# r-mafi/ClaraGenomicsAnalysis

Measured on AMD Instinct MI355X. Metric: POA windows/sec (consensus), higher is better.
Workload: dtype int16

## Files before the change

claragenomicsanalysis_amd/csrc/poa_batch.cpp:

```cpp
#include <claraparabricks/genomeworks/cudapoa/batch.hpp>
#include <claraparabricks/genomeworks/cudapoa/utils.hpp>

#include "gwamd_cudapoa.h"
#include "host_common.hpp"
#include "poa_batch_internal.hpp"
#include "poa_common.hpp"
#include "poa_plan.hpp"

#include <hip/hip_runtime.h>

#include <algorithm>
#include <cstdio>
#include <cstdlib>
#include <cstring>
#include <iomanip>
#include <sstream>
#include <string>

extern "C" hipError_t gwamd_internal_poa_launch(const gwamd::poa::Buffers* b, const gwamd::poa::Dims* d,
                                       const gwamd::poa::Scores* sc, int score_bits, int size_bits, int banded,
                                       int msa, hipStream_t stream);
extern "C" int gwamd_internal_poa_blocks_per_cu(const gwamd::poa::Dims* d, int score_bits, int size_bits, int banded,
                                                int msa);
extern "C" gwamd::poa::KernelRef gwamd_internal_poa_kernel(const gwamd::poa::Dims* d, int score_bits, int size_bits,
// ... 112 lines not shown
    }

    StatusType add_poa_group(std::vector<StatusType>& per_seq_status, const Group& poa_group) override
    {
        int32_t max_len = 0;
        for (const auto& e : poa_group)
            max_len = std::max(max_len, e.length);
        if (!reserve_buf(max_len))
            return StatusType::exceeded_maximum_poas;
        per_seq_status.clear();
        StatusType st = add_poa();
        if (st != StatusType::success)
            return st;
        for (const auto& e : poa_group)
            per_seq_status.push_back(add_seq_to_poa(e.seq, e.weights, e.length));
        return StatusType::success;
    }

    int32_t get_total_poas() const override { return poa_count_; }

    void generate_poa() override
    {
        if (poa_count_ == 0)
            return;
        upload();
        launch();
    }

    void upload()
    {
        ScopedDevice dev(device_id_);
        const size_t nb = num_bases_;
        GWAMD_HIP_CHECK(hipMemcpyAsync(d_seqs_.data(), h_seqs_.as<uint8_t>(), nb + 16, hipMemcpyHostToDevice, stream_));
        GWAMD_HIP_CHECK(hipMemcpyAsync(d_wts_.data(), h_wts_.as<int8_t>(), nb + 16, hipMemcpyHostToDevice, stream_));
        GWAMD_HIP_CHECK(hipMemcpyAsync(d_len_.data(), h_len_.as<int32_t>(), size_t(num_seqs_) * 4,
                                       hipMemcpyHostToDevice, stream_));
        GWAMD_HIP_CHECK(hipMemcpyAsync(d_off_.data(), h_off_.as<int64_t>(), size_t(num_seqs_) * 8,
                                       hipMemcpyHostToDevice, stream_));
        GWAMD_HIP_CHECK(hipMemcpyAsync(d_win_.data(), h_win_.as<gwamd::poa::WindowDesc>(),
                                       size_t(poa_count_) * sizeof(gwamd::poa::WindowDesc), hipMemcpyHostToDevice,
                                       stream_));
        bufs_.order = nullptr;
        bufs_.head  = nullptr;
        const auto kind = gwamd::poa::plan_window_order(h_win_.as<gwamd::poa::WindowDesc>(), h_len_.as<int32_t>(),
                                                        poa_count_, order_cus_, cap_.slots, dims_.lds_kernel != 0,
                                                        order_);
        if (kind == gwamd::poa::kNoOrder)
            return;
        const size_t order_b = size_t(poa_count_) * 4;
        h_order_.reserve(order_b, stream_);
        std::memcpy(h_order_.as<int32_t>(), order_.data(), order_b);
        int32_t* d_order = reinterpret_cast<int32_t*>(d_win_.data() + lay_.order_off);
        GWAMD_HIP_CHECK(hipMemcpyAsync(d_order, h_order_.as<int32_t>(), order_b, hipMemcpyHostToDevice, stream_));
        bufs_.order = d_order;
        if (kind == gwamd::poa::kOrderAndHead)
            bufs_.head = reinterpret_cast<int32_t*>(d_win_.data() + lay_.head_off);
    }

    void launch()
    {
        if (poa_count_ == 0)
            return;
        ScopedDevice dev(device_id_);
        gwamd::poa::Buffers b = bufs_;
        b.num_windows         = poa_count_;
        b.num_slots           = cap_.slots;
        if (b.head)
// ... 156 lines not shown

    void get_graphs(std::vector<DirectedGraph>& graphs, std::vector<StatusType>& output_status) override
    {
        fetch_graphs();
        graphs.resize(poa_count_);
        const size_t mn = size_t(dims_.max_nodes);
        for (int32_t w = 0; w < poa_count_; w++)
        {
            StatusType st = graph_status(w);
            output_status.push_back(st);
            if (st != StatusType::success)
                continue;
            DirectedGraph& g = graphs[w];
            for (int32_t v = 0; v < h_final_nodes_[w]; v++)
            {
                g.set_node_label(v, std::string(1, char(h_g_bases_[w * mn + v])));
                const int ne = h_g_in_cnt_[w * mn + v];
                for (int e = 0; e < ne; e++)
                {
                    size_t idx = (w * mn + v) * gwamd::poa::kMaxEdges + e;
                    g.add_edge(h_g_in_e_[idx], v, h_g_in_w_[idx]);
                }
            }
        }
    }

    int32_t batch_id() const override { return bid_; }

    void reset() override
    {
        poa_count_          = 0;
        num_bases_          = 0;
        num_seqs_           = 0;
        next_scores_offset_ = 0;
        avail_scorebuf_     = cap_.scorebuf_alloc;
        generated_          = false;
    }

    int32_t score_bits() const { return score_bits_; }
    int32_t size_bits() const { return size_bits_; }
    const gwamd::poa::Dims& dims() const { return dims_; }
    const std::vector<uint8_t>& host_cons() const { return h_cons_; }
    const std::vector<uint16_t>& host_cov() const { return h_cov_; }
    const std::vector<int32_t>& host_cons_len() const { return h_len_out_; }
    const std::vector<uint8_t>& host_status() const { return h_status_; }
    const std::vector<uint8_t>& host_msa() const { return h_msa_; }
    const std::vector<int32_t>& host_msa_len() const { return h_msa_len_; }
    const std::vector<uint8_t>& host_msa_status() const { return h_msa_status_; }
    const std::vector<uint8_t>& host_g_bases() const { return h_g_bases_; }
    const std::vector<uint16_t>& host_g_in_cnt() const { return h_g_in_cnt_; }
    const std::vector<int32_t>& host_g_in_e() const { return h_g_in_e_; }
    const std::vector<uint16_t>& host_g_in_w() const { return h_g_in_w_; }
    const std::vector<int32_t>& host_final_nodes() const { return h_final_nodes_; }
    int32_t window_num_seqs(int32_t w) const { return h_win_.as<const gwamd::poa::WindowDesc>()[w].num_seqs; }
    int8_t output_mask() const { return output_mask_; }
    int64_t device_bytes() const { return lay_.device_bytes(); }
    int32_t kernel_kind() const
    {
        return dims_.lds_kernel == 3 ? (dims_.band_ad ? 4 : 3) : (dims_.lds_kernel ? 2 : 1);
    }
    int32_t max_poas() const { return cap_.max_poas; }
    int32_t max_sequence_size() const { return bs_.max_sequence_size; }
    int32_t slots() const { return cap_.slots; }
    int32_t resident_slots() const { return cap_.resident; }
    void set_spoa_accurate(bool on) { dims_.spoa_accurate = on ? 1 : 0; }
    bool spoa_accurate() const { return dims_.spoa_accurate != 0; }
// ... 80 lines not shown
        return true;
    }

    StatusType add_poa()
    {
        if (poa_count_ == cap_.max_poas)
            return StatusType::exceeded_maximum_poas;
        h_win_.reserve(size_t(poa_count_ + 1) * sizeof(gwamd::poa::WindowDesc), stream_);
        gwamd::poa::WindowDesc& wd = h_win_.as<gwamd::poa::WindowDesc>()[poa_count_];
        wd.first_seq               = num_seqs_;
        wd.num_seqs                = 0;
        h_win_.used_               = size_t(poa_count_ + 1) * sizeof(gwamd::poa::WindowDesc);
        poa_count_++;
        generated_ = false;
        return StatusType::success;
    }

    StatusType add_seq_to_poa(const char* seq, const int8_t* weights, int32_t seq_len)
    {
        if (seq_len > bs_.max_sequence_size)
            return StatusType::exceeded_maximum_sequence_size;
        gwamd::poa::WindowDesc& wd = h_win_.as<gwamd::poa::WindowDesc>()[poa_count_ - 1];
        if (wd.num_seqs >= bs_.max_sequences_per_poa)
            return StatusType::exceeded_maximum_sequences_per_poa;
        if (weights != nullptr)
            for (int32_t i = 0; i < seq_len; i++)
                detail::check_non_negative(weights[i], "Base weights need to be non-negative");
        wd.num_seqs++;
        const size_t need = num_bases_ + size_t(seq_len) + 16;
        h_seqs_.reserve(need, stream_);
        h_wts_.reserve(need, stream_);
        if (seq_len > 0)
            std::memcpy(h_seqs_.as<uint8_t>() + num_bases_, seq, size_t(seq_len));
        if (weights == nullptr)
            std::memset(h_wts_.as<int8_t>() + num_bases_, 1, size_t(seq_len));
        else if (seq_len > 0)
            std::memcpy(h_wts_.as<int8_t>() + num_bases_, weights, size_t(seq_len));
        std::memset(h_seqs_.as<uint8_t>() + num_bases_ + seq_len, 0, 16);
        std::memset(h_wts_.as<int8_t>() + num_bases_ + seq_len, 0, 16);
        h_len_.reserve(size_t(num_seqs_ + 1) * 4, stream_);
        h_off_.reserve(size_t(num_seqs_ + 1) * 8, stream_);
        h_len_.as<int32_t>()[num_seqs_] = seq_len;
        h_off_.as<int64_t>()[num_seqs_] = int64_t(num_bases_);
        num_bases_ += size_t(seq_len);
        h_seqs_.used_ = h_wts_.used_ = num_bases_ + 16;
        num_seqs_++;
        h_len_.used_ = size_t(num_seqs_) * 4;
        h_off_.used_ = size_t(num_seqs_) * 8;
        return StatusType::success;
    }

    int32_t device_id_;
    hipStream_t stream_;
    int8_t output_mask_;
    BatchSize bs_;
    int16_t gap_, mismatch_, match_;
    bool banded_;
    int32_t score_bits_ = 16, size_bits_ = 16;
    gwamd::poa::PoaCapacity cap_;
    gwamd::poa::PoaLayout lay_;
    int32_t order_cus_ = 0;
    int64_t avail_scorebuf_ = 0, next_scores_offset_ = 0;
    int32_t poa_count_  = 0;
    int32_t num_seqs_   = 0;
    size_t num_bases_   = 0;
    bool generated_     = false;
    int32_t bid_        = 0;
    hipEvent_t ev_start_ = nullptr, ev_stop_ = nullptr;
    const gwamd::poa::PoaTuning tune_ = gwamd::poa::read_poa_tuning();
    gwamd::poa::Dims dims_{};
    std::vector<int32_t> order_;
    PinnedBuf h_order_;
    gwamd::poa::Buffers bufs_{};
    gwamd::host::DevBuf<uint8_t> d_seqs_, d_wts_, d_len_, d_off_, d_win_, d_slab_, d_codes_;
    PinnedBuf h_seqs_, h_wts_, h_len_, h_off_, h_win_;
    std::vector<uint8_t> h_cons_, h_status_, h_msa_, h_msa_status_, h_g_bases_, h_g_in_e_raw_;
    std::vector<uint16_t> h_cov_, h_g_in_cnt_, h_g_in_w_;
    std::vector<int32_t> h_len_out_, h_msa_len_, h_g_in_e_, h_final_nodes_;
    static int32_t batches_;
};

int32_t PoaBatch::batches_ = 0;

StatusType Init()
{
    int n = 0;
    if (hipGetDeviceCount(&n) != hipSuccess || n == 0)
        return StatusType::generic_error;
    return StatusType::success;
}

int64_t estimate_max_poas(const BatchSize& batch_size, bool banded_alignment, bool msa_flag,
                          size_t free_device_memory, float memory_usage_quota, int32_t mismatch_score,
                          int32_t gap_score, int32_t match_score)
{
    const size_t mem_per_batch = size_t(memory_usage_quota * double(free_device_memory));
    int64_t sizeof_score       = 2;
    int64_t per_poa            = 0;
// ... 625 lines not shown
```

claragenomicsanalysis_amd/csrc/poa_common.hpp:

```cpp
#pragma once

#include <cstddef>
#include <cstdint>

#include "poa_handover.hpp"

namespace gwamd
{
namespace poa
{

constexpr int kMaxEdges      = 50;
constexpr int kMaxAlignments = 50;
constexpr int kBandPad       = 8;
constexpr int kWave          = 64;
constexpr int kCellsPerLane  = 8;
constexpr int kChunk         = kWave * kCellsPerLane;
constexpr int kAdRing        = 128;
constexpr int kAdSpillDist   = kAdRing - kWave + 1;
constexpr int band_ring_rows(int cpl) { return cpl >= 16 ? 8 : 16; }
constexpr int band_tile_rows(int cpl) { return cpl >= 10 ? 32 : 64; }
constexpr int kReadGuard     = 64;
constexpr int kAdMaxWaves    = 4;
constexpr int kColShift      = 7;
// ... 34 lines not shown
    int32_t lds_bytes;
    int32_t lds_ring_off;
    int32_t lds_ring_rows;
    int32_t lds_sh_off;
    int32_t lds_rec_off;
    int32_t lds_xl_off;
    int32_t lds_xl_cap;
    int32_t lds_cpl;
    int32_t lds_waves;
    int32_t code_stride;
    int64_t aux_stride;
    int32_t aux_carry_off;
    int32_t lds_work_bytes;
    int32_t aux_reca_off;
    int32_t aux_recb_off;
    int32_t aux_col0_off;
    int32_t aux_flag_off;
    int32_t aux_xl_off;
    int32_t aux_xl_cap;
    int32_t aux_bx_off;
    int32_t aux_recc_off;
    int32_t aux_rece_off;
    int32_t band_ad;
    int32_t tb_rank;
    int32_t diag;
};

constexpr int kTbRanked     = 1;
constexpr int kTbStrips     = 2;
constexpr int kTbStrip32    = 4;
constexpr int kTbDefault    = kTbRanked | kTbStrips;
constexpr int kTbAboveShift = 3;
constexpr int kTbAboveMask  = 7;

constexpr int kDiagTopsortRing  = 1;
constexpr int kDiagFwdV1        = 2;
constexpr int kDiagTopsortFifo  = 4;
constexpr int kDiagRaconV1      = 8;
constexpr int kDiagConsensusHbm = 16;
constexpr int kDiagAddWave0     = 32;
constexpr int kDiagAddSerial    = 64;
constexpr int kDiagOrderKahn    = 128;
constexpr int kDiagSinkCap2     = 256;
constexpr int kDiagConsLdsShift = 16;

struct LdsShape
{
    int cpl, waves;
    bool wide;
};
constexpr LdsShape kLdsShapes[] = {{8, 1, true},   {8, 2, true},   {8, 4, true},   {8, 8, true},  {16, 8, true},
                                   {8, 1, false},  {16, 1, false}, {24, 1, false}, {32, 1, false}, {8, 2, false},
                                   {8, 3, false},  {8, 4, false},  {16, 4, false}, {4, 4, false}};
constexpr int kNumLdsShapes = int(sizeof(kLdsShapes) / sizeof(kLdsShapes[0]));

struct KernelRef
{
    const void* fn;
    int threads;
    size_t dynamic_lds;
};

constexpr int64_t lds_read_bytes(int64_t max_seq_len) { return (max_seq_len + 48 + 15) & ~int64_t(15); }

constexpr int kAddShBytes = 64;
constexpr int64_t lds_add_ms(int64_t max_seq_len) { return (max_seq_len + 16) & ~int64_t(15); }
// ... 121 lines not shown
```

claragenomicsanalysis_amd/csrc/poa_kernels.hip:

```cpp
#include <hip/hip_runtime.h>

#include <climits>
#include <cstdint>
#include <type_traits>
#include <utility>

#include "poa_wave.hpp"
#include "poa_order.hpp"
#include "poa_rowprog.hpp"

namespace gwamd
{
namespace poa
{

template <typename ScoreT, typename SizeT, bool BANDED, bool MSA>
__global__ void __launch_bounds__(kWave) poa_window_kernel(Buffers b, Dims d, Scores sc)
{
    extern __shared__ __align__(16) uint8_t lds_read[];
    __shared__ int sh_alen;
    __shared__ int sh_status;
    __shared__ int sh_len;

    const int w = b.order ? b.order[blockIdx.x] : int(blockIdx.x);
    if (w >= b.num_windows)
        return;
    const int lane = threadIdx.x;

    const WinGraph<SizeT> g     = bind_window<SizeT>(b, d.max_nodes, size_t(w));
    const SlotScratch<SizeT> sl = bind_slot<SizeT>(b, d, size_t(w));
    const WinMsa<SizeT> msa     = bind_window_msa<SizeT, MSA>(b, d, size_t(w));
    ScoreT* S       = static_cast<ScoreT*>(b.scores) + size_t(w) * d.score_rows * size_t(d.score_stride);
    SizeT *ag = sl.ag, *ar = sl.ar, *cpred = sl.cpred, *seq_begin = msa.seq_begin;
    int32_t* cscore = sl.cscore;
    uint16_t *ecov = msa.ecov, *ecovc = msa.ecov_cnt;

    PhaseTimer ph;
    const WindowDesc wd = b.windows[w];
    const int nseq      = wd.num_seqs;
    int status          = kSuccess;
    int64_t cells       = 0;
    int node_count      = 0;
// ... 658 lines not shown
                    if (2 * i + 1 == own_c)
                        endv = int(int16_t(E[i] >> 16));
                }
                const int v = L == 0 ? cin : __builtin_amdgcn_readlane(endv, own_lane);
                if (best_val < v)
                    best_val = v, best_row = r;
            }
#pragma unroll
            for (int i = 0; i < NR; i++)
                Eprev[i] = E[i];
            cin_prev = cin;
            rec_c    = rec_a;
            np_c     = np_a;
            pv_c     = pv_a;
            rec_a    = rec_b;
            np_a     = np_b;
            pv_a     = pv_b;
            rec_b    = uniform(int(rec_bb));
            GWAMD_FP_LAP(fp, 3);
        }
    }
    }
    if (nsweep > 1 || NW > 1)
    {
        GWAMD_LDS int* endp = (GWAMD_LDS int*)(shb + kShEnd);
        if (wave == own_span % NW && lane == 0)
            *endp = best_row;
        __syncthreads();
        best_row = uniform(*endp);
    }
    return best_row;
}

template <typename SizeT>
__device__ int traceback_codes(WinGraph<SizeT> g, const RowProg& P, int V, int L, int end_row,
                               const uint8_t* codes_f, int code_stride, uint8_t* tile_f, SizeT* ag_f, SizeT* ar_f,
                               int aln_cap, int lane, bool rank, int tbmode)
{
    g = as_global(g);
    const GWAMD_GLB uint8_t* codes = glb_of(codes_f);
    GWAMD_LDS uint8_t* tile        = lds_of(tile_f);
    GWAMD_GLB SizeT* ag            = glb_of(ag_f);
    GWAMD_GLB SizeT* ar            = glb_of(ar_f);
    const GWAMD_LDS uint32_t* prec = lds_of(P.rec);
    const GWAMD_LDS uint16_t* pxl  = lds_of(P.xl);

    V       = uniform(V);
    L       = uniform(L);
    int i   = uniform(end_row), j = L;
    int ti0 = INT_MIN / 2, tj0 = INT_MIN / 2;
    int n = 0, loops = 0;
    const int bound = L + V + 2;
    int eg = 0, er = 0;
    auto flush = [&](int upto) { tb_flush<SizeT>(g.sorted, ag, ar, aln_cap, upto, lane, eg, er); };
    auto load_tile = [&](int ii, int cj) {
        ti0 = max(0, ii - (kTileRows - 1));
        tj0 = max(0, cj - (kTileCols - 16)) & ~15;
        wave_sync();
        constexpr int kPer = kTileRows * (kTileCols / 16) / kWave;
        constexpr int kB   = 8;
#pragma unroll
        for (int b0 = 0; b0 < kPer; b0 += kB)
        {
            u32x4 v[kB];
#pragma unroll
            for (int u = 0; u < kB; u++)
            {
                const int t   = (b0 + u) * kWave + lane;
                const int tr  = t / (kTileCols / 16);
                const int tc  = (t % (kTileCols / 16)) * 16;
                const int rr  = ti0 + tr;
                const bool ok = rr <= V && tj0 + tc + 16 <= code_stride;
                v[u] = *reinterpret_cast<const GWAMD_GLB u32x4*>(codes + size_t(ok ? rr : 0) * code_stride +
                                                                 (ok ? tj0 + tc : 0));
                v[u] = ok ? v[u] : u32x4{0, 0, 0, 0};
            }
#pragma unroll
            for (int u = 0; u < kB; u++)
            {
                const int t  = (b0 + u) * kWave + lane;
                const int tr = t / (kTileCols / 16);
                const int tc = (t % (kTileCols / 16)) * 16;
                *reinterpret_cast<GWAMD_LDS u32x4*>(tile + tr * kTileCols + tc) = v[u];
            }
        }
        wave_sync();
    };
    constexpr uint32_t kSlow = 0xffffffffu;
    const bool win_ok        = V < 65535 && L < 65535;
    TbWin G;
    G.init(tbmode, i, L, kTileRows);
    uint32_t wpk0 = kSlow, wpk1 = kSlow;
    auto decode_cell = [&](int t) -> uint32_t {
        const int r  = G.row(t);
        const int c  = G.col(t);
        const int cj = c + kColShift;
        uint32_t res = kSlow;
        if (r >= 1 && c >= 0 && r >= ti0 && r < ti0 + kTileRows && cj >= tj0 && cj < tj0 + kTileCols)
        {
            const int code     = int(tile[(r - ti0) * kTileCols + (cj - tj0)]);
            const uint32_t rec = prec[r];
            const int dir      = code & 3;
            const int np       = int((rec >> 8) & 63);
            const int pj       = dir == 1 ? c : c - 1;
            if (pj < 0)
                res = kSlow;
            else if (dir == 2)
                res = (uint32_t(r) << 16) | uint32_t(pj);
            else if (np != int(kRecEscape))
            {
                const int p = np == 0 ? 0 : (np == 1 ? r - int(rec >> 16) : int(pxl[(rec >> 16) + (code >> 2)]));
                res         = (uint32_t(p) << 16) | uint32_t(pj);
            }
        }
        return res;
    };
    while (!(i == 0 && j == 0) && loops < bound)
    {
        i     = uniform(i);
// ... 50 lines not shown
            const int rec_v    = int(prec[i]);
            const int code     = uniform(code_v);
            const uint32_t rec = uint32_t(uniform(rec_v));
            const int dir      = code & 3;
            if (dir == 2)
            {
                pi = i;
                pj = j - 1;
            }
            else
            {
                const int np = int((rec >> 8) & 63), k = code >> 2;
                pi = np == 0 ? 0
                             : (np == 1 ? i - int(rec >> 16)
                                        : (np == int(kRecEscape) ? uniform(pred_row(g, int(g.sorted[i - 1]), k))
                                                                 : uniform(int(pxl[(rec >> 16) + k]))));
                pj = dir == 0 ? j - 1 : j;
            }
        }
        if (lane == (n & (kWave - 1)))
        {
            eg = i == pi ? -1 : i;
            er = j == pj ? -1 : j - 1;
        }
        n++;
        if ((n & (kWave - 1)) == 0)
            flush(n);
        i = pi;
        j = pj;
    }
    if ((n & (kWave - 1)) != 0)
        flush(n);
    wave_sync();
    if (loops >= bound || n > aln_cap)
        return -1;
    return n;
}

#include "poa_fwd2.hpp"
#include "poa_fwd_w.hpp"

template <bool MSA, int CPL, int NW, bool W>
__global__ void __launch_bounds__(kWave * NW, W ? (NW >= 8 ? 2 : 1) : (NW >= 4 ? 2 : 1))
    poa_window_kernel_lds(Buffers b, Dims d, Scores sc)
{
    using SizeT  = int16_t;
    using RowT   = typename std::conditional<W, int32_t, int16_t>::type;
    extern __shared__ __align__(16) uint8_t lds[];
    __shared__ int sh_status;
    __shared__ int sh_len;

    __shared__ int sh_next;
    if (int(blockIdx.x) >= b.num_windows)
        return;
    const int tid      = threadIdx.x;
    const int lane     = tid & (kWave - 1);
    const int wave     = uniform(tid / kWave);
    constexpr int kThr = kWave * NW;
    const size_t slot  = blockIdx.x;

    uint8_t* lread   = lds;
    RowT* ring       = reinterpret_cast<RowT*>(lds + d.lds_ring_off);
    uint8_t* tile    = lds + d.lds_ring_off;
    const int rstride = d.score_stride;
    GWAMD_LDS uint8_t* shb = (GWAMD_LDS uint8_t*)(lds) + d.lds_sh_off;
    const AddScratch AX = lds_add_scratch((GWAMD_LDS uint8_t*)(lds) + d.lds_ring_off, d.max_seq_len, d.max_nodes,
                                          false, (GWAMD_LDS int*)(shb));
    const bool add_fits = lds_add_fits(d.max_seq_len, d.max_nodes, d.lds_rec_off - d.lds_ring_off);
    const int add_mode  = (d.diag & kDiagAddSerial) ? 2 : (((d.diag & kDiagAddWave0) || !add_fits) ? 1 : 0);

    for (int idx = blockIdx.x; idx < b.num_windows;)
    {
    const int w     = b.order ? b.order[idx] : idx;
    const WinGraph<SizeT> g     = bind_window<SizeT>(b, d.max_nodes, size_t(w));
    const SlotScratch<SizeT> sl = bind_slot<SizeT>(b, d, slot);
    const WinMsa<SizeT> msa     = bind_window_msa<SizeT, MSA>(b, d, size_t(w));
    SizeT *ag = sl.ag, *ar = sl.ar, *cpred = sl.cpred, *seq_begin = msa.seq_begin;
    int32_t* cscore = sl.cscore;
    uint16_t *ecov = msa.ecov, *ecovc = msa.ecov_cnt;
    RowT* spill      = static_cast<RowT*>(b.scores) + slot * d.score_rows * size_t(rstride);
    uint8_t* codes   = b.codes + slot * size_t(d.aux_stride);
    uint32_t* rec    = reinterpret_cast<uint32_t*>(lds + d.lds_rec_off);
    uint16_t* xl     = reinterpret_cast<uint16_t*>(lds + d.lds_xl_off);
    RowT* carry      = reinterpret_cast<RowT*>(codes + d.aux_carry_off);
    RowProg P{rec, xl, d.lds_ring_rows - 1};

    PhaseTimer ph;
    FwdProf fp;
    const bool use_v2 = !W && fwd2_ok(sc) && !(d.diag & kDiagFwdV1);
    const WindowDesc wd = b.windows[w];
    const int nseq      = wd.num_seqs;
    int status          = kSuccess;
    int64_t cells       = 0;
    int node_count      = 0;
    int lv_hint         = 0;
    bool order_kahn = true;
    bool splice_on  = !d.spoa_accurate && !(d.diag & (kDiagTopsortFifo | kDiagOrderKahn));
    int tie_hold    = 0;
    const int sink_cap = (d.diag & kDiagSinkCap2) ? 2 : kSinkCap;
    const int xcap  = d.lds_xl_cap - kSinkWords;
    GWAMD_LDS uint16_t* sinks = (GWAMD_LDS uint16_t*)(lds + d.lds_xl_off) + xcap;
    int32_t* ostat  = b.order_stats + size_t(w) * kOrderStats;
    auto count      = [&](int k) {
        if (tid == 0)
            __hip_atomic_fetch_add(ostat + k, 1, __ATOMIC_RELAXED, __HIP_MEMORY_SCOPE_AGENT);
    };
    if (tid < kOrderStats)
        ostat[tid] = 0;
    auto kahn_sort = [&](WinGraph<SizeT> gx, int n, int n_prev) {
        const bool done = topsort_levels<SizeT, NW>(gx, n, n_prev, (GWAMD_LDS uint8_t*)(lds), d.lds_sh_off, tid,
                                                    kThr, cpred, lv_hint);
        if (!done && tid == 0)
            topsort_kahn<SizeT>(gx, n, cscore);
        lv_hint = done ? n : 0;
        __syncthreads();
    };

    if (nseq > 0)
    {
        const int len0      = b.seq_len[wd.first_seq];
        const uint8_t* seq0 = b.seqs + b.seq_off[wd.first_seq];
// ... 125 lines not shown
                if (code == 2 && !order_kahn)
                {
                    const size_t mn    = size_t(d.max_nodes);
                    WinGraph<SizeT> gk = g;
                    gk.sorted          = cpred + mn;
                    gk.pos             = cpred + 2 * mn;
                    for (int i = tid; i < V; i += kThr)
                        glb(gk.sorted)[i] = glb(g.sorted)[i];
                    kahn_sort(gk, V, V);
                    count(kOsTieSorts);
                    if (wave == 0)
                    {
                        int kp = INT_MAX;
                        if (tied)
                            kp = int(glb(gk.pos)[int(glb(g.sorted)[srow_l - 1])]);
                        const int kmin = -wave_max(-kp);
                        const uint64_t m = __builtin_amdgcn_ballot_w64(kp == kmin);
                        const int er   = __builtin_amdgcn_readlane(srow_l, uniform(__builtin_ctzll(m)));
                        if (lane == 0)
                            sh_len = er;
                    }
                    __syncthreads();
                    end_row = uniform(sh_len);
                    __syncthreads();
                    stage_and_program_w0();
                    __syncthreads();
                }
                tie_hold = code == 2 ? 2 : max(tie_hold - 1, 0);
            }
            else if (tie_hold > 0)
                tie_hold--;
            if (wave == 0)
            {
                const int alen_w = traceback_codes<SizeT>(g, P, V, L, end_row, codes, d.code_stride, tile, ag, ar,
                                                          d.aln_cap, lane, (d.tb_rank & kTbRanked) != 0,
                                                          d.tb_rank);
                if (lane == 0)
                    sh_len = alen_w;
            }
            __syncthreads();
            const int alen = uniform(sh_len);
            __syncthreads();
            ph.lap<kPhTraceback>();
            if (alen == -1)
            {
                status = kLoopCountExceeded;
                break;
            }
            int add_r = -1;
            if (add_mode == 0)
                add_r = add_alignment_waves<MSA, NW, NW + (W ? 16 : 0)>(lds_kernel_args(), w, int(slot), s, off,
                                                                        node_count, alen, L,
                                                                        (GWAMD_LDS uint8_t*)(lds));
            if (wave == 0)
            {
                int nc = node_count;
                int rc = -1;
                if (add_mode == 0)
                {
                    nc = add_r >> 8;
                    rc = (add_r & 0xff) == 0xff ? -1 : (add_r & 0xff);
                }
                else if (add_mode == 1)
                    rc = add_alignment_parallel<SizeT, MSA>(g, nc, ag, ar, alen, L, lread, wts_g, s, ecov, ecovc,
                                                            seq_begin, d.max_seqs, AX, lane);
                if (rc < 0)
                {
                    if (lane == 0)
                    {
// ... 65 lines not shown
                }
                ph.lap<kPhTopsort>();
                wave_sync();
                if (lane == 0)
                {
                    sh_status = rc;
                    sh_len    = nc;
                }
            }
            __syncthreads();
            status     = uniform(sh_status);
            node_count = uniform(sh_len);
            __syncthreads();
            if (status != kSuccess)
                break;
        }
    }
    if (wave == 0)
    {
        finish_window<SizeT, MSA, NW>(b, d, w, lane, g, status, nseq, node_count, cscore, cpred, ecov, ecovc,
                                      seq_begin, sh_len, sh_status, (GWAMD_LDS uint8_t*)(lds), d.lds_sh_off);
        ph.lap<kPhOutput>();
        if (lane == 0)
        {
            if (b.phase)
            {
                ph.store(b.phase + size_t(w) * kPhases);
#ifdef GWAMD_FWD_PROFILE
                const int slot[8] = {kPhBackbone, kPhAdd, kPhTopsort, kPhOutput, kPhForward, kPhTraceback, kPhRowProg,
                                     kPhTotal};
                for (int i = 0; i < 8; i++)
                    b.phase[size_t(w) * kPhases + slot[i]] = int64_t(fp.t[i]);
#endif
            }
            b.final_nodes[w] = node_count;
            b.cells[w]       = cells;
        }
    }
#if defined(GWAMD_FWD_PROFILE) && defined(GWAMD_FWD_PROFILE_WAVE)
    __syncthreads();
    if (wave == GWAMD_FWD_PROFILE_WAVE && lane == 0 && b.phase)
    {
        const int slot[8] = {kPhBackbone, kPhAdd, kPhTopsort, kPhOutput, kPhForward, kPhTraceback, kPhRowProg,
                             kPhTotal};
        for (int i = 0; i < 8; i++)
            b.phase[size_t(w) * kPhases + slot[i]] = int64_t(fp.t[i]);
    }
#endif
    if (b.head == nullptr)
        break;
    __syncthreads();
    if (tid == 0)
        sh_next = b.num_slots + atomicAdd(b.head, 1);
    __syncthreads();
    idx = uniform(sh_next);
    }
}

}
}

extern "C" gwamd::poa::KernelRef gwamd_internal_poa_band_kernel(const gwamd::poa::Dims* d, int score_bits,
                                                                int size_bits, int msa);

namespace
{
// ... 90 lines not shown
```

claragenomicsanalysis_amd/csrc/poa_tuning.hpp:

```cpp
#pragma once

#include "diag_env.hpp"
#include "poa_common.hpp"

#include <algorithm>
#include <cstdio>
#include <cstdlib>
#include <cstring>

namespace gwamd
{
namespace poa
{

struct PoaTuning
{
    bool force_v1     = false;
    bool lds_shape    = false;
    int lds_cpl       = 0;
    int lds_waves     = 0;
    int lds_pad       = 0;
    int band_fwd      = 0;
    int band_ad_waves = kAdMaxWaves;
    int tb_rank       = kTbDefault;
// ... 17 lines not shown
                                   {"GWAMD_TB_WALK", "scalar_strip32", kTbStrips | kTbStrip32}};
    static const Choice kDiag[] = {{"GWAMD_TOPSORT_RING", nullptr, kDiagTopsortRing},
                                   {"GWAMD_POA_FWD", "v1", kDiagFwdV1},
                                   {"GWAMD_TOPSORT", "fifo", kDiagTopsortFifo},
                                   {"GWAMD_RACON", "v1", kDiagRaconV1},
                                   {"GWAMD_CONSENSUS", "hbm", kDiagConsensusHbm},
                                   {"GWAMD_POA_ADD", "wave0", kDiagAddWave0},
                                   {"GWAMD_POA_ADD", "serial", kDiagAddSerial},
                                   {"GWAMD_POA_ORDER", "kahn", kDiagOrderKahn},
                                   {"GWAMD_POA_SINK_CAP", "2", kDiagSinkCap2}};
    static const Choice kFwd[]  = {{"GWAMD_BAND_FWD", "ad", 1}, {"GWAMD_BAND_FWD", "row", 2}};
    auto is = [](const Choice& c) {
        const char* v = diag_env(c.name);
        return v && (c.value ? std::strcmp(v, c.value) == 0 : std::atoi(v) != 0);
    };
    auto number = [](const char* name, int unset) {
        const char* v = diag_env(name);
        return v ? std::atoi(v) : unset;
    };
    PoaTuning t;
    t.force_v1 = is({"GWAMD_POA_KERNEL", "v1", 0});
    if (const char* sh = diag_env("GWAMD_POA_LDS_SHAPE"))
        t.lds_shape = std::sscanf(sh, "%d,%d", &t.lds_cpl, &t.lds_waves) == 2;
    t.lds_pad = number("GWAMD_POA_LDS_PAD", 0);
    for (const Choice& c : kFwd)
        if (is(c))
            t.band_fwd = c.bits;
    t.band_ad_waves = std::max(1, std::min(kAdMaxWaves, number("GWAMD_BAND_AD_WAVES", kAdMaxWaves)));
    for (const Choice& c : kWalk)
        if (is(c))
            t.tb_rank = c.bits;
    if (diag_env("GWAMD_TB_ABOVE"))
        t.tb_rank |= (std::min(std::max(number("GWAMD_TB_ABOVE", 0), 0), 6) + 1) << kTbAboveShift;
    for (const Choice& c : kDiag)
        if (is(c))
            t.diag |= c.bits;
    if (diag_env("GWAMD_CONSENSUS_LDS_BYTES"))
        t.diag |= int(uint32_t(std::min(std::max(number("GWAMD_CONSENSUS_LDS_BYTES", 0), 1), 65535)) << kDiagConsLdsShift);
    t.slots     = std::max(0, number("GWAMD_POA_SLOTS", 0));
    t.order_cus = std::max(0, number("GWAMD_LAUNCH_ORDER_CUS", 0));
    return t;
}

}
}
```

claragenomicsanalysis_amd/csrc/poa_wave.hpp:

```cpp
#pragma once

#include <hip/hip_runtime.h>

#include <climits>
#include <cstdint>
#include <type_traits>

#include "poa_device.hpp"

#define GWAMD_LDS __attribute__((address_space(3)))
#define GWAMD_GLB __attribute__((address_space(1)))

#include "poa_consensus.hpp"

namespace gwamd
{
namespace poa
{

template <typename T>
__device__ __forceinline__ GWAMD_LDS T* lds_of(T* p)
{
    return (GWAMD_LDS T*)(uintptr_t)(uint32_t)(uintptr_t)(p);
}
// ... 2373 lines not shown
    cl += steps;
}

template <int kCmin, typename Flush>
__device__ __forceinline__ void walk_window_scalar(uint32_t wpk0, uint32_t wpk1, const TbWin& G, int& ci, int& cj,
                                                   int& cn, int& cl, int bound, int lane, int& eg, int& er,
                                                   GWAMD_LDS uint8_t*, Flush&& flush)
{
    constexpr uint32_t kSlow = 0xffffffffu;
    while (true)
    {
        const int idx     = G.index(ci, cj);
        const uint32_t nx = uint32_t(idx < kWave ? __builtin_amdgcn_readlane(int(wpk0), idx)
                                                 : __builtin_amdgcn_readlane(int(wpk1), idx - kWave));
        if (nx == kSlow)
            break;
        const int pi = int(nx >> 16), pj = int(nx & 0xffffu);
        cl++;
        if (lane == (cn & (kWave - 1)))
        {
            eg = ci == pi ? -1 : ci;
            er = cj == pj ? -1 : cj - 1;
        }
        cn++;
        if ((cn & (kWave - 1)) == 0)
            flush(cn);
        ci = pi;
        cj = pj;
        if ((ci == 0 && cj == 0) || cl >= bound || ci < 1 || (kCmin > 0 && cj < kCmin) || G.index(ci, cj) < 0)
            break;
    }
}

template <typename SizeT, typename SortedP, typename PairP>
__device__ __forceinline__ void tb_flush(SortedP sorted, PairP ag, PairP ar, int aln_cap, int upto, int lane, int eg,
                                         int er)
{
    const int base = (upto - 1) & ~(kWave - 1);
    const int k    = base + lane;
    if (k < upto && k < aln_cap)
    {
        ag[k] = SizeT(eg > 0 ? int(sorted[eg - 1]) : -1);
        ar[k] = SizeT(er);
    }
}

}
}
```

Baseline: 21430.

## Stage traceback codes through an async LDS band ring with prefetch

```diff
diff --git a/claragenomicsanalysis_amd/csrc/poa_batch.cpp b/claragenomicsanalysis_amd/csrc/poa_batch.cpp
--- a/claragenomicsanalysis_amd/csrc/poa_batch.cpp
+++ b/claragenomicsanalysis_amd/csrc/poa_batch.cpp
@@ -168,7 +168,15 @@
         ScopedDevice dev(device_id_);
         const size_t nb = num_bases_;
         GWAMD_HIP_CHECK(hipMemcpyAsync(d_seqs_.data(), h_seqs_.as<uint8_t>(), nb + 16, hipMemcpyHostToDevice, stream_));
-        GWAMD_HIP_CHECK(hipMemcpyAsync(d_wts_.data(), h_wts_.as<int8_t>(), nb + 16, hipMemcpyHostToDevice, stream_));
+        if (any_weights_)
+            GWAMD_HIP_CHECK(hipMemcpyAsync(d_wts_.data(), h_wts_.as<int8_t>(), nb + 16, hipMemcpyHostToDevice,
+                                           stream_));
+        else
+        {
+            if (nb > 0)
+                GWAMD_HIP_CHECK(hipMemsetAsync(d_wts_.data(), 1, nb, stream_));
+            GWAMD_HIP_CHECK(hipMemsetAsync(d_wts_.data() + nb, 0, 16, stream_));
+        }
         GWAMD_HIP_CHECK(hipMemcpyAsync(d_len_.data(), h_len_.as<int32_t>(), size_t(num_seqs_) * 4,
                                        hipMemcpyHostToDevice, stream_));
         GWAMD_HIP_CHECK(hipMemcpyAsync(d_off_.data(), h_off_.as<int64_t>(), size_t(num_seqs_) * 8,
@@ -391,6 +399,7 @@
         poa_count_          = 0;
         num_bases_          = 0;
         num_seqs_           = 0;
+        any_weights_        = false;
         next_scores_offset_ = 0;
         avail_scorebuf_     = cap_.scorebuf_alloc;
         generated_          = false;
@@ -537,12 +546,20 @@
         h_wts_.reserve(need, stream_);
         if (seq_len > 0)
             std::memcpy(h_seqs_.as<uint8_t>() + num_bases_, seq, size_t(seq_len));
-        if (weights == nullptr)
-            std::memset(h_wts_.as<int8_t>() + num_bases_, 1, size_t(seq_len));
-        else if (seq_len > 0)
-            std::memcpy(h_wts_.as<int8_t>() + num_bases_, weights, size_t(seq_len));
+        if (weights != nullptr && !any_weights_)
+        {
+            std::memset(h_wts_.as<int8_t>(), 1, num_bases_);
+            any_weights_ = true;
+        }
+        if (any_weights_)
+        {
+            if (weights == nullptr)
+                std::memset(h_wts_.as<int8_t>() + num_bases_, 1, size_t(seq_len));
+            else if (seq_len > 0)
+                std::memcpy(h_wts_.as<int8_t>() + num_bases_, weights, size_t(seq_len));
+            std::memset(h_wts_.as<int8_t>() + num_bases_ + seq_len, 0, 16);
+        }
         std::memset(h_seqs_.as<uint8_t>() + num_bases_ + seq_len, 0, 16);
-        std::memset(h_wts_.as<int8_t>() + num_bases_ + seq_len, 0, 16);
         h_len_.reserve(size_t(num_seqs_ + 1) * 4, stream_);
         h_off_.reserve(size_t(num_seqs_ + 1) * 8, stream_);
         h_len_.as<int32_t>()[num_seqs_] = seq_len;
@@ -569,6 +586,7 @@
     int32_t poa_count_  = 0;
     int32_t num_seqs_   = 0;
     size_t num_bases_   = 0;
+    bool any_weights_   = false;
     bool generated_     = false;
     int32_t bid_        = 0;
     hipEvent_t ev_start_ = nullptr, ev_stop_ = nullptr;
diff --git a/claragenomicsanalysis_amd/csrc/poa_common.hpp b/claragenomicsanalysis_amd/csrc/poa_common.hpp
--- a/claragenomicsanalysis_amd/csrc/poa_common.hpp
+++ b/claragenomicsanalysis_amd/csrc/poa_common.hpp
@@ -90,6 +90,8 @@
 constexpr int kTbDefault    = kTbRanked | kTbStrips;
 constexpr int kTbAboveShift = 3;
 constexpr int kTbAboveMask  = 7;
+constexpr int kTbStageTile  = 64;
+constexpr int kTbStageMiss  = 128;
 
 constexpr int kDiagTopsortRing  = 1;
 constexpr int kDiagFwdV1        = 2;
diff --git a/claragenomicsanalysis_amd/csrc/poa_kernels.hip b/claragenomicsanalysis_amd/csrc/poa_kernels.hip
--- a/claragenomicsanalysis_amd/csrc/poa_kernels.hip
+++ b/claragenomicsanalysis_amd/csrc/poa_kernels.hip
@@ -8,6 +8,7 @@
 #include "poa_wave.hpp"
 #include "poa_order.hpp"
 #include "poa_rowprog.hpp"
+#include "poa_tbring.hpp"
 
 namespace gwamd
 {
@@ -732,11 +733,41 @@
     return best_row;
 }
 
+#ifdef GWAMD_TB_PROFILE
+struct TbProf
+{
+    uint64_t tile = 0, flush = 0, total = 0;
+    uint64_t tiles = 0, flushes = 0, reads = 0;
+    uint64_t m = 0;
+    __device__ __forceinline__ void mark()
+    {
+        asm volatile("" ::: "memory");
+        m = __builtin_amdgcn_s_memtime();
+    }
+    __device__ __forceinline__ uint64_t since(bool lds)
+    {
+        if (lds)
+            asm volatile("s_waitcnt lgkmcnt(0)" ::: "memory");
+        else
+            asm volatile("" ::: "memory");
+        return __builtin_amdgcn_s_memtime() - m;
+    }
+};
+#define GWAMD_TBP_PARAM , TbProf& tp
+#define GWAMD_TBP_ARG , tp
+#define GWAMD_TBP(stmt) stmt
+#else
+#define GWAMD_TBP_PARAM
+#define GWAMD_TBP_ARG
+#define GWAMD_TBP(stmt)
+#endif
+
 template <typename SizeT>
 __device__ int traceback_codes(WinGraph<SizeT> g, const RowProg& P, int V, int L, int end_row,
                                const uint8_t* codes_f, int code_stride, uint8_t* tile_f, SizeT* ag_f, SizeT* ar_f,
-                               int aln_cap, int lane, bool rank, int tbmode)
-{
+                               int aln_cap, int lane, bool rank, int tbmode GWAMD_TBP_PARAM)
+{
+    GWAMD_TBP(const uint64_t tp_t0 = __builtin_amdgcn_s_memtime());
     g = as_global(g);
     const GWAMD_GLB uint8_t* codes = glb_of(codes_f);
     GWAMD_LDS uint8_t* tile        = lds_of(tile_f);
@@ -752,8 +783,13 @@
     int n = 0, loops = 0;
     const int bound = L + V + 2;
     int eg = 0, er = 0;
-    auto flush = [&](int upto) { tb_flush<SizeT>(g.sorted, ag, ar, aln_cap, upto, lane, eg, er); };
+    auto flush = [&](int upto) {
+        GWAMD_TBP(tp.mark());
+        tb_flush<SizeT>(g.sorted, ag, ar, aln_cap, upto, lane, eg, er);
+        GWAMD_TBP(tp.flush += tp.since(false); tp.flushes++);
+    };
     auto load_tile = [&](int ii, int cj) {
+        GWAMD_TBP(tp.mark());
         ti0 = max(0, ii - (kTileRows - 1));
         tj0 = max(0, cj - (kTileCols - 16)) & ~15;
         wave_sync();
@@ -785,6 +821,7 @@
             }
         }
         wave_sync();
+        GWAMD_TBP(tp.tile += tp.since(true); tp.tiles++);
     };
     constexpr uint32_t kSlow = 0xffffffffu;
     const bool win_ok        = V < 65535 && L < 65535;
@@ -901,6 +938,260 @@
     if ((n & (kWave - 1)) != 0)
         flush(n);
     wave_sync();
+    GWAMD_TBP(tp.total += __builtin_amdgcn_s_memtime() - tp_t0; tp.reads++);
+    if (loops >= bound || n > aln_cap)
+        return -1;
+    return n;
+}
+
+__device__ __forceinline__ void tb_load_lds16(const GWAMD_GLB uint8_t* src, uint32_t lds_dst)
+{
+    uint32_t keep;
+    asm volatile("s_mov_b32 %0, m0\n\ts_mov_b32 m0, %2\n\ts_nop 0\n\tglobal_load_lds_dwordx4 %1, off\n\ts_mov_b32 m0, %0"
+                 : "=&s"(keep)
+                 : "v"(src), "s"(lds_dst)
+                 : "memory");
+}
+
+struct TbRing
+{
+    const GWAMD_GLB uint8_t* codes;
+    int stride, V, lane, skew_;
+    uint32_t lds_base;
+    uint32_t meta_v = tbring::kEmpty;
+    int seq_v       = 0;
+    uint32_t pend   = 0;
+    int issued      = 0;
+    __device__ __forceinline__ uint32_t meta(int slot) const
+    {
+        return uint32_t(__builtin_amdgcn_readlane(int(meta_v), uniform(slot)));
+    }
+    __device__ __forceinline__ uint32_t pending() const { return pend; }
+    __device__ __forceinline__ int skew() const { return skew_; }
+    __device__ __forceinline__ void wait_for(uint32_t slots)
+    {
+        int newest = 0;
+        for (uint32_t m = slots; m; m &= m - 1)
+            newest = max(newest, __builtin_amdgcn_readlane(seq_v, uniform(__builtin_ctz(m))));
+        switch (min(issued - newest, 6))
+        {
+        case 0: asm volatile("s_waitcnt vmcnt(0)" ::: "memory"); break;
+        case 1: asm volatile("s_waitcnt vmcnt(2)" ::: "memory"); break;
+        case 2: asm volatile("s_waitcnt vmcnt(4)" ::: "memory"); break;
+        case 3: asm volatile("s_waitcnt vmcnt(6)" ::: "memory"); break;
+        case 4: asm volatile("s_waitcnt vmcnt(8)" ::: "memory"); break;
+        case 5: asm volatile("s_waitcnt vmcnt(10)" ::: "memory"); break;
+        default: asm volatile("s_waitcnt vmcnt(12)" ::: "memory"); break;
+        }
+        static_assert(tbring::kSlotLoads == 2, "vmcnt per slot");
+        pend &= ~uint32_t(__builtin_amdgcn_ballot_w64(lane < tbring::kSlots && seq_v <= newest));
+    }
+    __device__ __forceinline__ void wait_all()
+    {
+        asm volatile("s_waitcnt vmcnt(0)" ::: "memory");
+        pend = 0;
+    }
+    __device__ __forceinline__ void stage(int band, int origin)
+    {
+        const int slot = uniform(tbring::slot_of(band));
+        meta_v         = lane == slot ? tbring::pack(band, origin) : meta_v;
+        issued++;
+        seq_v = lane == slot ? issued : seq_v;
+        pend |= 1u << slot;
+        asm volatile("s_waitcnt lgkmcnt(0)" ::: "memory");
+#pragma unroll
+        for (int k = 0; k < tbring::kSlotLoads; k++)
+        {
+            const int r = tbring::src_row(band, k, lane, V);
+            const int c = tbring::src_col(origin, lane, stride);
+            tb_load_lds16(codes + size_t(r) * size_t(stride) + size_t(c),
+                          lds_base + uint32_t(slot * tbring::kSlotBytes + k * (tbring::kSlotBytes / tbring::kSlotLoads)));
+        }
+    }
+};
+
+template <typename SizeT>
+__device__ int traceback_codes_ring(WinGraph<SizeT> g, const RowProg& P, int V, int L, int end_row,
+                                    const uint8_t* codes_f, int code_stride, uint8_t* tile_f, SizeT* ag_f,
+                                    SizeT* ar_f, int aln_cap, int lane, bool rank, int tbmode GWAMD_TBP_PARAM)
+{
+    namespace tr = tbring;
+    GWAMD_TBP(const uint64_t tp_t0 = __builtin_amdgcn_s_memtime());
+    g = as_global(g);
+    const GWAMD_GLB uint8_t* codes = glb_of(codes_f);
+    GWAMD_LDS uint8_t* tile        = lds_of(tile_f);
+    GWAMD_GLB SizeT* ag            = glb_of(ag_f);
+    GWAMD_GLB SizeT* ar            = glb_of(ar_f);
+    const GWAMD_LDS uint32_t* prec = lds_of(P.rec);
+    const GWAMD_LDS uint16_t* pxl  = lds_of(P.xl);
+
+    V     = uniform(V);
+    L     = uniform(L);
+    int i = uniform(end_row), j = L;
+    int n = 0, loops = 0;
+    const int bound = L + V + 2;
+    int eg = 0, er = 0;
+    TbRing R;
+    R.codes    = codes;
+    R.stride   = uniform(code_stride);
+    R.V        = V;
+    R.lane     = lane;
+    R.skew_    = (tbmode & kTbStageMiss) ? tr::kCols : 0;
+    R.lds_base = uint32_t(uniform(int((uint32_t)(uintptr_t)tile)));
+    auto flush = [&](int upto) {
+        GWAMD_TBP(tp.mark());
+        tb_flush<SizeT, true>(g.sorted, ag, ar, aln_cap, upto, lane, eg, er);
+        GWAMD_TBP(tp.flush += tp.since(false); tp.flushes++);
+    };
+    constexpr uint32_t kSlow = 0xffffffffu;
+    const bool win_ok        = V < 65535 && L < 65535;
+    TbWin G;
+    G.init(tbmode, i, L, tr::kMaxWindowRows);
+    uint32_t wpk0 = kSlow, wpk1 = kSlow;
+    auto decode_cell = [&](int t) -> uint32_t {
+        const int r  = G.row(t);
+        const int c  = G.col(t);
+        const int cj = c + kColShift;
+        const uint32_t m = uint32_t(
+            __builtin_amdgcn_ds_bpermute(tr::slot_of(tr::band_of(max(r, 0))) * 4, int(R.meta_v)));
+        uint32_t res = kSlow;
+        if (r >= 1 && c >= 0 && r <= V && cj < R.stride && tr::covers_cell(m, r, cj))
+        {
+            const int code     = int(tile[tr::cell_offset(m, r, cj)]);
+            const uint32_t rec = prec[r];
+            const int dir      = code & 3;
+            const int np       = int((rec >> 8) & 63);
+            const int pj       = dir == 1 ? c : c - 1;
+            if (pj < 0)
+                res = kSlow;
+            else if (dir == 2)
+                res = (uint32_t(r) << 16) | uint32_t(pj);
+            else if (np != int(kRecEscape))
+            {
+                const int p = np == 0 ? 0 : (np == 1 ? r - int(rec >> 16) : int(pxl[(rec >> 16) + (code >> 2)]));
+                res         = (uint32_t(p) << 16) | uint32_t(pj);
+            }
+        }
+        return res;
+    };
+    while (!(i == 0 && j == 0) && loops < bound)
+    {
+        i       = uniform(i);
+        j       = uniform(j);
+        n       = uniform(n);
+        loops   = uniform(loops);
+        R.pend   = uint32_t(uniform(int(R.pend)));
+        R.issued = uniform(R.issued);
+        G.wi0   = uniform(G.wi0);
+        G.wj0   = uniform(G.wj0);
+        G.slope = uniform(G.slope);
+        G.next  = uniform(G.next);
+        if (win_ok && i >= 1)
+        {
+            if (G.index(i, j) < 0)
+            {
+                G.refill(i, j);
+                const int cj   = j + kColShift;
+                const int r_lo = max(i - G.row_span(), 1), c_lo = max(cj - G.col_span(), 0);
+                GWAMD_TBP(tp.mark());
+                const int staged = tr::cover_or_stage(R, r_lo, i, c_lo, cj, i, cj, G.slope, R.stride);
+                GWAMD_TBP(tp.tile += tp.since(true); tp.tiles += staged);
+                wpk0 = decode_cell(lane);
+                wpk1 = decode_cell(lane + kWave);
+                GWAMD_TBP(tp.mark());
+                tr::fill_ahead(R, i, cj, r_lo, G.slope, R.stride);
+                GWAMD_TBP(tp.tile += tp.since(false));
+            }
+            int ci = i, cj = j, cn = n, cl = loops;
+            if (rank)
+                walk_window_ranked<0>(wpk0, wpk1, G, ci, cj, cn, cl, bound, lane, eg, er, tile + tr::kRingBytes,
+                                      flush);
+            else
+                walk_window_scalar<0>(wpk0, wpk1, G, ci, cj, cn, cl, bound, lane, eg, er, nullptr, flush);
+            if (cl != loops)
+            {
+                G.follow(ci, cj);
+                i     = ci;
+                j     = cj;
+                n     = cn;
+                loops = cl;
+                continue;
+            }
+        }
+        loops++;
+        int pi, pj;
+        if (i == 0)
+        {
+            pi = 0;
+            pj = j - 1;
+        }
+        else
+        {
+            const int cj = j + kColShift;
+            GWAMD_TBP(tp.mark());
+            const int staged = tr::cover_or_stage(R, i, i, cj, cj, i, cj, G.slope, R.stride);
+            GWAMD_TBP(tp.tile += tp.since(true); tp.tiles += staged);
+            const uint32_t m   = R.meta(tr::slot_of(tr::band_of(i)));
+            const int code_v   = int(tile[tr::cell_offset(m, i, cj)]);
+            const int rec_v    = int(prec[i]);
+            const int code     = uniform(code_v);
+            const uint32_t rec = uint32_t(uniform(rec_v));
+            const int dir      = code & 3;
+            if (dir == 2)
+            {
+                pi = i;
+                pj = j - 1;
+            }
+            else
+            {
+                const int np = int((rec >> 8) & 63), k = code >> 2;
+                pi = np == 0 ? 0
+                             : (np == 1 ? i - int(rec >> 16)
+                                        : (np == int(kRecEscape) ? uniform(pred_row(g, int(g.sorted[i - 1]), k))
+                                                                 : uniform(int(pxl[(rec >> 16) + k]))));
+                pj = dir == 0 ? j - 1 : j;
+            }
+        }
+        if (lane == (n & (kWave - 1)))
+        {
+            eg = i == pi ? -1 : i;
+            er = j == pj ? -1 : j - 1;
+        }
+        n++;
+        if ((n & (kWave - 1)) == 0)
+            flush(n);
+        i = pi;
+        j = pj;
+    }
+    if ((n & (kWave - 1)) != 0)
+        flush(n);
+    R.wait_all();
+    wave_sync();
+    GWAMD_TBP(tp.mark());
+    const int nn = min(n, aln_cap);
+    for (int k0 = 0; k0 < nn; k0 += 8 * kWave)
+    {
+        int v[8];
+#pragma unroll
+        for (int u = 0; u < 8; u++)
+            v[u] = int(ag[min(k0 + u * kWave + lane, nn - 1)]);
+#pragma unroll
+        for (int u = 0; u < 8; u++)
+        {
+            const int node = int(g.sorted[max(v[u], 1) - 1]);
+            v[u]           = v[u] > 0 ? node : -1;
+        }
+#pragma unroll
+        for (int u = 0; u < 8; u++)
+        {
+            const int k = k0 + u * kWave + lane;
+            if (k < nn)
+                ag[k] = SizeT(v[u]);
+        }
+    }
+    wave_sync();
+    GWAMD_TBP(tp.flush += tp.since(false));
+    GWAMD_TBP(tp.total += __builtin_amdgcn_s_memtime() - tp_t0; tp.reads++);
     if (loops >= bound || n > aln_cap)
         return -1;
     return n;
@@ -956,6 +1247,7 @@
 
     PhaseTimer ph;
     FwdProf fp;
+    GWAMD_TBP(TbProf tp);
     const bool use_v2 = !W && fwd2_ok(sc) && !(d.diag & kDiagFwdV1);
     const WindowDesc wd = b.windows[w];
     const int nseq      = wd.num_seqs;
@@ -1147,9 +1439,13 @@
                 tie_hold--;
             if (wave == 0)
             {
-                const int alen_w = traceback_codes<SizeT>(g, P, V, L, end_row, codes, d.code_stride, tile, ag, ar,
-                                                          d.aln_cap, lane, (d.tb_rank & kTbRanked) != 0,
-                                                          d.tb_rank);
+                const bool tb_ranked = (d.tb_rank & kTbRanked) != 0;
+                const int alen_w =
+                    (d.tb_rank & kTbStageTile)
+                        ? traceback_codes<SizeT>(g, P, V, L, end_row, codes, d.code_stride, tile, ag, ar, d.aln_cap,
+                                                 lane, tb_ranked, d.tb_rank GWAMD_TBP_ARG)
+                        : traceback_codes_ring<SizeT>(g, P, V, L, end_row, codes, d.code_stride, tile, ag, ar,
+                                                      d.aln_cap, lane, tb_ranked, d.tb_rank GWAMD_TBP_ARG);
                 if (lane == 0)
                     sh_len = alen_w;
             }
@@ -1281,6 +1577,15 @@
                 for (int i = 0; i < 8; i++)
                     b.phase[size_t(w) * kPhases + slot[i]] = int64_t(fp.t[i]);
 #endif
+#ifdef GWAMD_TB_PROFILE
+                int64_t* ph8     = b.phase + size_t(w) * kPhases;
+                ph8[kPhBackbone] = int64_t(tp.tile);
+                ph8[kPhAdd]      = int64_t(tp.flush);
+                ph8[kPhTopsort]  = int64_t(tp.total);
+                ph8[kPhOutput]   = int64_t(tp.tiles);
+                ph8[kPhRowProg]  = int64_t(tp.flushes);
+                ph8[kPhForward]  = int64_t(tp.reads);
+#endif
             }
             b.final_nodes[w] = node_count;
             b.cells[w]       = cells;
diff --git a/claragenomicsanalysis_amd/csrc/poa_tbring.hpp b/claragenomicsanalysis_amd/csrc/poa_tbring.hpp
--- /dev/null
+++ b/claragenomicsanalysis_amd/csrc/poa_tbring.hpp
@@ -0,0 +1,143 @@
+#pragma once
+
+#include <cstdint>
+
+#if defined(__HIPCC__)
+#define GWAMD_TBR_FN __host__ __device__ __forceinline__
+#else
+#define GWAMD_TBR_FN inline
+#endif
+
+namespace gwamd
+{
+namespace poa
+{
+namespace tbring
+{
+
+constexpr int kBandShift = 4;
+constexpr int kBandRows  = 1 << kBandShift;
+constexpr int kSlots     = 8;
+constexpr int kCols      = 128;
+constexpr int kPiece     = 16;
+constexpr int kSlotBytes = kBandRows * kCols;
+constexpr int kSlotLoads = kSlotBytes / (64 * kPiece);
+constexpr int kRingBytes = kSlots * kSlotBytes;
+constexpr int kMinAhead  = 2;
+constexpr uint32_t kEmpty = 0xffffffffu;
+static_assert(kSlotLoads == 2, "a slot is two wave loads");
+
+constexpr int kMaxWindowRows = (kSlots - kMinAhead - 1) * kBandRows + 1;
+static_assert(1 + (kMaxWindowRows - 1 + kBandRows - 1) / kBandRows == kSlots - kMinAhead, "window bands");
+
+GWAMD_TBR_FN int band_of(int r) { return r >> kBandShift; }
+GWAMD_TBR_FN int slot_of(int band) { return band & (kSlots - 1); }
+GWAMD_TBR_FN int band_mid_row(int band) { return (band << kBandShift) + kBandRows / 2; }
+GWAMD_TBR_FN uint32_t pack(int band, int origin) { return (uint32_t(band) << 16) | uint32_t(origin); }
+GWAMD_TBR_FN int meta_band(uint32_t m) { return int(m >> 16); }
+GWAMD_TBR_FN int meta_origin(uint32_t m) { return int(m & 0xffffu); }
+
+GWAMD_TBR_FN int max_origin(int stride) { return stride > kCols ? stride - kCols : 0; }
+
+GWAMD_TBR_FN int origin_at(int c, int stride)
+{
+    const int o  = (c - kCols / 2) & ~(kPiece - 1);
+    const int hi = max_origin(stride);
+    return o < 0 ? 0 : (o > hi ? hi : o);
+}
+
+GWAMD_TBR_FN int origin_covering(int want, int c_lo, int c_hi, int stride)
+{
+    const int lo = (c_hi - (kCols - 1) + (kPiece - 1)) & ~(kPiece - 1);
+    const int hi = c_lo & ~(kPiece - 1);
+    int o        = want < lo ? lo : (want > hi ? hi : want);
+    const int mx = max_origin(stride);
+    o            = o > mx ? mx : o;
+    return o < 0 ? 0 : o;
+}
+
+GWAMD_TBR_FN bool covers(uint32_t m, int band, int c_lo, int c_hi)
+{
+    const int o = meta_origin(m);
+    return m != kEmpty && meta_band(m) == band && o <= c_lo && c_hi < o + kCols;
+}
+GWAMD_TBR_FN bool covers_cell(uint32_t m, int r, int c) { return covers(m, band_of(r), c, c); }
+
+GWAMD_TBR_FN int cell_offset(uint32_t m, int r, int c)
+{
+    return slot_of(band_of(r)) * kSlotBytes + (r & (kBandRows - 1)) * kCols + (c - meta_origin(m));
+}
+
+GWAMD_TBR_FN int predict_col(int i, int c, int r, int slope16)
+{
+    return c - ((i - r) * 16) / (slope16 > 0 ? slope16 : 16);
+}
+
+GWAMD_TBR_FN int band_floor(int i)
+{
+    const int b = band_of(i) - (kSlots - 1);
+    return b < 0 ? 0 : b;
+}
+
+GWAMD_TBR_FN int src_row(int band, int k, int lane, int V)
+{
+    const int r = (band << kBandShift) + k * (kBandRows / kSlotLoads) + lane / (kCols / kPiece);
+    return r > V ? V : r;
+}
+GWAMD_TBR_FN int src_col(int origin, int lane, int stride)
+{
+    const int c = origin + (lane % (kCols / kPiece)) * kPiece;
+    return c > stride - kPiece ? stride - kPiece : c;
+}
+
+
+template <class Ring>
+GWAMD_TBR_FN int cover_or_stage(Ring& R, int r_lo, int r_hi, int c_lo, int c_hi, int i, int c, int slope16,
+                                int stride)
+{
+    const int b_lo = band_of(r_lo), b_hi = band_of(r_hi);
+    uint32_t need = 0, miss = 0;
+    for (int b = b_hi; b >= b_lo; b--)
+    {
+        const int s = slot_of(b);
+        need |= 1u << s;
+        if (!covers(R.meta(s), b, c_lo, c_hi))
+            miss |= 1u << s;
+    }
+    int staged = 0;
+    if (miss)
+    {
+        if (R.pending())
+            R.wait_for(R.pending());
+        for (int b = b_hi; b >= b_lo; b--)
+            if ((miss >> slot_of(b)) & 1u)
+            {
+                const int want = origin_at(predict_col(i, c, band_mid_row(b), slope16) + R.skew(), stride);
+                R.stage(b, origin_covering(want, c_lo, c_hi, stride));
+                staged++;
+            }
+    }
+    if (R.pending() & need)
+        R.wait_for(R.pending() & need);
+    return staged;
+}
+
+template <class Ring>
+GWAMD_TBR_FN int fill_ahead(Ring& R, int i, int c, int r_lo, int slope16, int stride)
+{
+    int issued = 0;
+    for (int b = band_of(r_lo) - 1; b >= band_floor(i); b--)
+    {
+        const int s      = slot_of(b);
+        const uint32_t m = R.meta(s);
+        if (((R.pending() >> s) & 1u) || (m != kEmpty && meta_band(m) == b))
+            continue;
+        R.stage(b, origin_at(predict_col(i, c, band_mid_row(b), slope16) + R.skew(), stride));
+        issued++;
+    }
+    return issued;
+}
+
+}
+}
+}
diff --git a/claragenomicsanalysis_amd/csrc/poa_tuning.hpp b/claragenomicsanalysis_amd/csrc/poa_tuning.hpp
--- a/claragenomicsanalysis_amd/csrc/poa_tuning.hpp
+++ b/claragenomicsanalysis_amd/csrc/poa_tuning.hpp
@@ -73,6 +73,9 @@
             t.tb_rank = c.bits;
     if (diag_env("GWAMD_TB_ABOVE"))
         t.tb_rank |= (std::min(std::max(number("GWAMD_TB_ABOVE", 0), 0), 6) + 1) << kTbAboveShift;
+    for (const Choice& c : {Choice{"GWAMD_TB_STAGE", "tile", kTbStageTile}, Choice{"GWAMD_TB_STAGE", "miss", kTbStageMiss}})
+        if (is(c))
+            t.tb_rank |= c.bits;
     for (const Choice& c : kDiag)
         if (is(c))
             t.diag |= c.bits;
diff --git a/claragenomicsanalysis_amd/csrc/poa_wave.hpp b/claragenomicsanalysis_amd/csrc/poa_wave.hpp
--- a/claragenomicsanalysis_amd/csrc/poa_wave.hpp
+++ b/claragenomicsanalysis_amd/csrc/poa_wave.hpp
@@ -2429,7 +2429,7 @@
     }
 }
 
-template <typename SizeT, typename SortedP, typename PairP>
+template <typename SizeT, bool kRows = false, typename SortedP, typename PairP>
 __device__ __forceinline__ void tb_flush(SortedP sorted, PairP ag, PairP ar, int aln_cap, int upto, int lane, int eg,
                                          int er)
 {
@@ -2437,7 +2437,7 @@
     const int k    = base + lane;
     if (k < upto && k < aln_cap)
     {
-        ag[k] = SizeT(eg > 0 ? int(sorted[eg - 1]) : -1);
+        ag[k] = SizeT(eg > 0 ? (kRows ? eg : int(sorted[eg - 1])) : -1);
         ar[k] = SizeT(er);
     }
 }
```

New measurement: 20880. 0.974x the previous value.
